# LittleWat/multichannel-semseg-with-uda

Hardware: AMD Instinct MI355X
Metric: RGB-D img/s (6x480x640) MCD train step, drn_d_38 (higher is better)
Workload: dtype f32 (operands split 2-way into scaled fp16, 3 cross terms on the fp16 MFMA pipe, fp32 accumulate)

## Files before the change

include/mcdseg.h:

```cpp
#ifndef MCDSEG_H
#define MCDSEG_H

#include <stddef.h>
#include <stdint.h>

#ifdef __cplusplus
extern "C" {
#endif
#pragma GCC visibility push(default)

#define MCDSEG_VERSION 101

int mcdseg_version(void);
const char* mcdseg_last_error(void);

#define MCDSEG_COMM_ID_BYTES 128
int mcdseg_comm_unique_id(void* id128);
int mcdseg_comm_init(void** comm, int32_t nranks, const void* id128, int32_t rank);
int mcdseg_comm_destroy(void* comm);
int mcdseg_allreduce(float* buf, int64_t count, void* comm, void* stream);

int32_t mcdseg_option_count(void);
const char* mcdseg_option_name(int32_t index);
int mcdseg_set_option(const char* name, int64_t value);
// ... 18 lines not shown
int mcdseg_conv_dgrad(const mcdseg_conv_desc* d, const float* dy, const float* wp_dgrad, float* dx, void* stream);
#define MCDSEG_MATH_F16X3 3
#define MCDSEG_MATH_BF16X6 6
#define MCDSEG_MATH_F16X1 1
int mcdseg_conv_split_packed_bytes(const mcdseg_conv_desc* d, int32_t math, int64_t* fprop_bytes, int64_t* dgrad_bytes);
int32_t mcdseg_conv_split_direct_ok(const mcdseg_conv_desc* d);
int64_t mcdseg_conv_split_stat_rows(const mcdseg_conv_desc* d);
int64_t mcdseg_conv_split_stat_rows_for(const mcdseg_conv_desc* d, int32_t math, int32_t presplit);
int32_t mcdseg_conv_split_window_ok(const mcdseg_conv_desc* d, int32_t math, int32_t presplit, int32_t dgrad);
int32_t mcdseg_conv_split_tile_config(int32_t M, int64_t P, int32_t presplit);
int mcdseg_absmax(const float* x, int64_t n, float* bound, void* stream);
int mcdseg_conv_split_pack_weights(const mcdseg_conv_desc* d, int32_t math, const float* w, void* wp_fprop, void* wp_dgrad,
                                   float* w_bound, void* stream);
int mcdseg_conv_split_pack_weights_multi(const int64_t* ptrs, const int32_t* dims, int32_t n, int32_t math, float* bounds,
                                         void* stream);
int mcdseg_conv_split_fprop(const mcdseg_conv_desc* d, int32_t math, const float* x, const void* x_cb, const float* x_bound,
                            const void* wp_fprop, const float* w_bound, const float* bias, float* y, float* stat_partials,
                            void* stream);
int mcdseg_conv_split_fprop_affine(const mcdseg_conv_desc* d, int32_t math, const float* x, const void* x_cb, const float* x_bound,
                                   const void* wp_fprop, const float* w_bound, const float* scale, const float* shift,
                                   const float* residual, int32_t relu, float* y, void* stream);
int mcdseg_conv_split_dgrad(const mcdseg_conv_desc* d, int32_t math, const float* dy, const void* dy_cb, const float* dy_bound,
                            const void* wp_dgrad, const float* w_bound, float* dx, void* stream);
int mcdseg_conv_split_dgrad_add(const mcdseg_conv_desc* d, int32_t math, const float* dy, const void* dy_cb, const float* dy_bound,
                                const void* wp_dgrad, const float* w_bound, const float* addend, float* dx, int32_t part, void* stream);
int64_t mcdseg_conv_split_parts(const mcdseg_conv_desc* d, int32_t math, int32_t presplit, int32_t dgrad);
int32_t mcdseg_conv_split_rest_pingpong(const mcdseg_conv_desc* d, int32_t math, int32_t presplit, int32_t dgrad);
int32_t mcdseg_conv_split_wide_pingpong(const mcdseg_conv_desc* d, int32_t math, int32_t presplit, int32_t dgrad);
int mcdseg_conv_split_fprop_part(const mcdseg_conv_desc* d, int32_t math, const float* x, const void* x_cb, const float* x_bound,
                                 const void* wp_fprop, const float* w_bound, const float* bias, float* y, float* stat_partials,
// ... 141 lines not shown
                         int32_t relu, void* stream);
size_t mcdseg_bn_bwd_half_workspace_bytes(int32_t N, int32_t C, int32_t HW);
int mcdseg_bn_bwd_reduce_half(const void* dy16, const void* y_cb, const void* z16, const float* z_bound, const float* mean,
                              const float* rstd, const float* gamma, const float* beta, float* dgamma, float* dbeta, float* dz_bound,
                              int32_t mask_kind, int32_t train, int32_t N, int32_t C, int32_t HW, void* workspace, size_t workspace_bytes,
                              void* stream);
int mcdseg_bn_bwd_apply_half(const void* dy16, const void* y_cb, const void* z16, const float* z_bound, const float* mean,
                             const float* rstd, const float* gamma, const float* beta, const float* dgamma, const float* dbeta, void* dz_cb,
                             const float* dz_bound, void* dres16, int32_t mask_kind, int32_t train, int32_t N, int32_t C, int32_t HW,
                             void* stream);
int mcdseg_pack_bf16_units(const float* x, void* out16, int32_t N, int32_t C, int32_t HW, void* stream);
int mcdseg_unpack_bf16_units(const void* in16, float* x, int32_t N, int32_t C, int32_t HW, void* stream);

int mcdseg_sgd_momentum_flat(float* p, const float* g, float* v, int64_t n, float lr, float momentum,
                             float weight_decay, float grad_scale, void* stream);

int mcdseg_adam_flat(float* p, const float* g, float* m, float* v, int64_t n, float lr_over_bc1, float beta1, float beta2,
                     float inv_sqrt_bc2, float eps, float weight_decay, float grad_scale, void* stream);

#pragma GCC visibility pop
#ifdef __cplusplus
}
#endif
#endif
```

multichannel-semseg-with-uda_amd/csrc/conv_gemm_split.hip:

```cpp
#include <cstdlib>
#include <type_traits>

#include "conv_split_params.h"
#include "options.h"

namespace {


template <class P, int WM, int WN, int WAVES_M, int WAVES_N, bool DGRAD, bool PRESPLIT>
__global__ __launch_bounds__(256, 2) void conv_gemm_split_kernel(ConvSplitParams p) {
  constexpr int BM = 32 * WM * WAVES_M;
  constexpr int BN = 32 * WN * WAVES_N;
  constexpr int NT = 256;
  static_assert(WAVES_M * WAVES_N == 4, "4 waves per workgroup");
  constexpr int B_ITEMS = BN * 2 / NT;
  constexpr int NP = P::NP;
  constexpr int NQ = 2 * NP;
  typedef typename P::frag frag;
  constexpr int A_CHUNKS = NQ * BM;
  constexpr int A_ITERS = (A_CHUNKS + NT - 1) / NT;
  constexpr bool A_EXACT = (A_CHUNKS % NT) == 0;
  constexpr bool A_DMA = A_EXACT;
  constexpr int A_ITERS_DMA = ((2 * P::NPU * BM) % NT == 0) ? (2 * P::NPU * BM) / NT : A_ITERS;
  constexpr int A_BYTES = NQ * BM * 16, B_BYTES = NQ * BN * 16;
// ... 679 lines not shown
      m = t > m ? t : m;
    }
    i += n4 << 2;
  }
  for (; i < n; i += step) {
    const unsigned b = __float_as_uint(x[i]) & 0x7FFFFFFFu;
    m = b > m ? b : m;
  }
  for (int o = 1; o < 64; o <<= 1) {
    const unsigned t = __shfl_xor(m, o);
    m = t > m ? t : m;
  }
  if ((threadIdx.x & 63) == 0 && m != 0u) atomicMax(out, m);
}

__global__ __launch_bounds__(256) void absmax_multi_kernel(const int64_t* __restrict__ ptrs, const int32_t* __restrict__ dims) {
  const int e = blockIdx.y;
  const float* __restrict__ x = reinterpret_cast<const float*>(ptrs[4 * e + 0]);
  unsigned* __restrict__ out = reinterpret_cast<unsigned*>(ptrs[4 * e + 3]);
  const int64_t n = (int64_t)dims[4 * e + 0] * dims[4 * e + 1] * dims[4 * e + 2];
  const int64_t step = (int64_t)gridDim.x * blockDim.x;
  unsigned m = 0u;
  int64_t i = blockIdx.x * (int64_t)blockDim.x + threadIdx.x;
  for (; i + 3 * step < n; i += 4 * step) {
    const unsigned b0 = __float_as_uint(x[i]) & 0x7FFFFFFFu, b1 = __float_as_uint(x[i + step]) & 0x7FFFFFFFu;
    const unsigned b2 = __float_as_uint(x[i + 2 * step]) & 0x7FFFFFFFu, b3 = __float_as_uint(x[i + 3 * step]) & 0x7FFFFFFFu;
    const unsigned c0 = b0 > b1 ? b0 : b1, c1 = b2 > b3 ? b2 : b3;
    const unsigned c = c0 > c1 ? c0 : c1;
    m = c > m ? c : m;
  }
  for (; i < n; i += step) {
    const unsigned b = __float_as_uint(x[i]) & 0x7FFFFFFFu;
    m = b > m ? b : m;
  }
  for (int o = 1; o < 64; o <<= 1) {
    const unsigned t = __shfl_xor(m, o);
    m = t > m ? t : m;
  }
  if ((threadIdx.x & 63) == 0 && m != 0u) atomicMax(out, m);
}

template <class P>
__global__ __launch_bounds__(256) void pack_weights_multi_kernel(const int64_t* __restrict__ ptrs, const int32_t* __restrict__ dims) {
  constexpr int NP = P::NP;
  __shared__ float tile[32 * 16 * 9 + 32];
  const int e = blockIdx.y >> 1, mode = blockIdx.y & 1;
  const float* __restrict__ w = reinterpret_cast<const float*>(ptrs[4 * e + 0]);
  typename P::elem* __restrict__ out = reinterpret_cast<typename P::elem*>(ptrs[4 * e + 1 + mode]);
  if (out == nullptr) return;
  const float inv_scale = 1.f / operand_scale<P>(reinterpret_cast<const float*>(ptrs[4 * e + 3]));
  const int Cout = dims[4 * e + 0], Cin = dims[4 * e + 1], T = dims[4 * e + 2];
  const int M = mode == 0 ? Cout : Cin;
  const int K = mode == 0 ? Cin : Cout;
  const int Mp = M <= 32 ? 32 : (M <= 64 ? 64 : ((M + 127) / 128) * 128);
  const int Kp = ((K + 15) / 16) * 16;
  const int MT = T <= 9 ? 32 : (T <= 18 ? 16 : (T <= 36 ? 8 : 4));
  const int row_len = 16 * T + 1;
  const int m_tiles = Mp / MT, chunks = Kp / 16;
  const int t = threadIdx.x;
  for (int tl = blockIdx.x; tl < m_tiles * chunks; tl += gridDim.x) {
    const int chunk = tl / m_tiles, m0 = (tl - chunk * m_tiles) * MT, k0 = chunk * 16;
    __syncthreads();
    if (mode == 0) {
      for (int idx = t; idx < MT * 16 * T; idx += 256) {
        const int mm = idx / (16 * T), col = idx - mm * (16 * T);
// ... 240 lines not shown
                       (__bf16*)wp_dgrad, (const float*)nullptr, d->Cout, d->Cin, T);
  MCD_LAUNCH_CHECK("conv_split_pack_weights");
  return 0;
}

extern "C" int mcdseg_conv_split_pack_weights_multi(const int64_t* ptrs, const int32_t* dims, int32_t n, int32_t math, float* bounds,
                                                    void* stream) {
  math = mcd_storage_math(math);
  MCD_REQUIRE(ptrs && dims && n > 0 && n <= 32767, "conv_split_pack_weights_multi: bad table");
  MCD_REQUIRE(math == MCDSEG_MATH_BF16X6 || math == MCDSEG_MATH_F16X3, "conv_split_pack_weights_multi: unknown math %d", math);
  MCD_REQUIRE(math != MCDSEG_MATH_F16X3 || bounds != nullptr, "conv_split_pack_weights_multi: f16x3 needs the bounds array");
  hipStream_t st = (hipStream_t)stream;
  const unsigned pack_blocks = (unsigned)(mcd_opt(MCD_OPT_PACK_BLOCKS) > 0 ? mcd_opt(MCD_OPT_PACK_BLOCKS) : 192);
  if (math == MCDSEG_MATH_F16X3) {
    (void)hipMemsetAsync(bounds, 0, sizeof(float) * (size_t)n, st);
    hipLaunchKernelGGL(absmax_multi_kernel, dim3(48, (unsigned)n), dim3(256), 0, st, ptrs, dims);
    MCD_LAUNCH_CHECK("absmax_multi");
    hipLaunchKernelGGL(pack_weights_multi_kernel<SplitF16x3>, dim3(pack_blocks, 2u * (unsigned)n), dim3(256), 0, st, ptrs, dims);
  } else {
    hipLaunchKernelGGL(pack_weights_multi_kernel<SplitBf16x6>, dim3(pack_blocks, 2u * (unsigned)n), dim3(256), 0, st, ptrs, dims);
  }
  MCD_LAUNCH_CHECK("conv_split_pack_weights_multi");
  return 0;
}

static int split_cb_bytes(const mcdseg_conv_desc* d, int math, int C, int HW, const void* cb, int* piece_bytes, long long* piece_stride) {
  *piece_bytes = 0;
  *piece_stride = 0;
  if (cb == nullptr) return 0;
  MCD_REQUIRE((C % 8) == 0, "conv_split: a pre-split operand needs a channel count divisible by 8 (got %d)", C);
  MCD_REQUIRE(d->Ncb == 0 || d->Ncb >= d->N, "conv_split: Ncb (%d) must be 0 or at least N (%d)", d->Ncb, d->N);
  const int64_t b = (int64_t)d->N * C * HW * 2;
  MCD_REQUIRE(b < (1ll << 31), "conv_split: one piece of the pre-split operand exceeds 2 GiB; split the batch");
  *piece_bytes = (int)b;
  *piece_stride = math == MCDSEG_MATH_F16X1 ? 0 : (long long)(d->Ncb ? d->Ncb : d->N) * C * HW * 2;
  return 0;
}

// ... 217 lines not shown
```

multichannel-semseg-with-uda_amd/csrc/sgd.hip:

```cpp
#include "common.h"

namespace {

__global__ __launch_bounds__(256) void sgd_momentum_kernel(float* __restrict__ p, const float* __restrict__ g, float* __restrict__ v,
                                                           int64_t n4, int64_t n, float lr, float mu, float wd, float gs) {
  float4* p4 = reinterpret_cast<float4*>(p);
  const float4* g4 = reinterpret_cast<const float4*>(g);
  float4* v4 = reinterpret_cast<float4*>(v);
  for (int64_t i = blockIdx.x * (int64_t)blockDim.x + threadIdx.x; i < n4; i += (int64_t)gridDim.x * blockDim.x) {
    float4 pp = p4[i];
    const float4 gg = g4[i];
    float4 vv = v4[i];
    vv.x = fmaf(mu, vv.x, fmaf(wd, pp.x, gg.x * gs));
    vv.y = fmaf(mu, vv.y, fmaf(wd, pp.y, gg.y * gs));
    vv.z = fmaf(mu, vv.z, fmaf(wd, pp.z, gg.z * gs));
    vv.w = fmaf(mu, vv.w, fmaf(wd, pp.w, gg.w * gs));
    pp.x = fmaf(-lr, vv.x, pp.x);
    pp.y = fmaf(-lr, vv.y, pp.y);
    pp.z = fmaf(-lr, vv.z, pp.z);
    pp.w = fmaf(-lr, vv.w, pp.w);
    v4[i] = vv;
    p4[i] = pp;
  }
  for (int64_t i = n4 * 4 + blockIdx.x * (int64_t)blockDim.x + threadIdx.x; i < n; i += (int64_t)gridDim.x * blockDim.x) {
// ... 6 lines not shown
}

extern "C" int mcdseg_sgd_momentum_flat(float* p, const float* g, float* v, int64_t n, float lr, float momentum, float weight_decay,
                                        float grad_scale, void* stream) {
  MCD_REQUIRE(p && g && v && n >= 0, "sgd_momentum_flat: bad arguments");
  if (n == 0) return 0;
  const bool al = ((reinterpret_cast<uintptr_t>(p) | reinterpret_cast<uintptr_t>(g) | reinterpret_cast<uintptr_t>(v)) & 15) == 0;
  const int64_t n4 = al ? n / 4 : 0;
  int64_t blocks = ceil_div64(n4 > 0 ? n4 : n, 256);
  if (blocks > 2048) blocks = 2048;
  hipLaunchKernelGGL(sgd_momentum_kernel, dim3((unsigned)blocks), dim3(256), 0, (hipStream_t)stream, p, g, v, n4, n, lr, momentum,
                     weight_decay, grad_scale);
  MCD_LAUNCH_CHECK("sgd_momentum_flat");
  return 0;
}
```

multichannel-semseg-with-uda_amd/mcdseg/_lib.py:

```python
import ctypes
import glob
import os
import subprocess
import threading

HERE = os.path.dirname(os.path.abspath(__file__))
PKG = os.path.dirname(HERE)
REPO = os.path.dirname(PKG)
CSRC = os.path.join(PKG, "csrc")
INCLUDE = os.path.join(REPO, "include")
LIB_PATH = os.environ.get("MCDSEG_LIB") or os.path.join(HERE, "libmcdseg.so")

c_void_p, c_int, c_i32, c_i64, c_float, c_size_t = (ctypes.c_void_p, ctypes.c_int, ctypes.c_int32, ctypes.c_int64,
                                                    ctypes.c_float, ctypes.c_size_t)


class ConvDesc(ctypes.Structure):
    _fields_ = [(n, c_i32) for n in ("N", "Cin", "H", "W", "Cout", "KH", "KW", "stride", "pad", "dil", "Ho", "Wo", "Ncb")]


_P = ctypes.POINTER
_SIGNATURES = {
    "mcdseg_version": (c_int, []),
    "mcdseg_last_error": (ctypes.c_char_p, []),
# ... 13 lines not shown
    "mcdseg_conv_split_window_ok": (c_i32, [_P(ConvDesc), c_i32, c_i32, c_i32]),
    "mcdseg_conv_split_direct_ok": (c_i32, [_P(ConvDesc)]),
    "mcdseg_conv_split_tile_config": (c_i32, [c_i32, c_i64, c_i32]),
    "mcdseg_conv_fprop": (c_int, [_P(ConvDesc), c_void_p, c_void_p, c_void_p, c_void_p, c_void_p, c_void_p]),
    "mcdseg_conv_fprop_affine": (c_int, [_P(ConvDesc), c_void_p, c_void_p, c_void_p, c_void_p, c_void_p, c_i32, c_void_p, c_void_p]),
    "mcdseg_bn_eval_affine": (c_int, [c_void_p] * 5 + [c_i32, c_float, c_void_p, c_void_p, c_void_p]),
    "mcdseg_predict_workspace_bytes": (c_size_t, [c_i32, c_i32]),
    "mcdseg_predict_labels": (c_int, [c_void_p] * 4 + [c_i32] * 4 + [c_void_p, c_size_t, c_void_p]),
    "mcdseg_predict_up8_workspace_bytes": (c_size_t, [c_i32, c_i32]),
    "mcdseg_predict_labels_up8": (c_int, [c_void_p] * 4 + [c_i32] * 5 + [c_void_p, c_size_t, c_void_p]),
    "mcdseg_depth_image_u8": (c_int, [c_void_p, c_void_p] + [c_i32] * 4 + [c_void_p]),
    "mcdseg_absmax": (c_int, [c_void_p, c_i64, c_void_p, c_void_p]),
    "mcdseg_conv_split_packed_bytes": (c_int, [_P(ConvDesc), c_i32, _P(c_i64), _P(c_i64)]),
    "mcdseg_conv_split_pack_weights": (c_int, [_P(ConvDesc), c_i32] + [c_void_p] * 5),
    "mcdseg_conv_split_pack_weights_multi": (c_int, [c_void_p, c_void_p, c_i32, c_i32, c_void_p, c_void_p]),
    "mcdseg_conv_split_fprop": (c_int, [_P(ConvDesc), c_i32] + [c_void_p] * 9),
    "mcdseg_conv_split_fprop_affine": (c_int, [_P(ConvDesc), c_i32] + [c_void_p] * 8 + [c_i32, c_void_p, c_void_p]),
    "mcdseg_conv_split_dgrad": (c_int, [_P(ConvDesc), c_i32] + [c_void_p] * 7),
    "mcdseg_conv_split_parts": (c_i64, [_P(ConvDesc), c_i32, c_i32, c_i32]),
    "mcdseg_conv_split_rest_pingpong": (c_i32, [_P(ConvDesc), c_i32, c_i32, c_i32]),
    "mcdseg_conv_split_wide_pingpong": (c_i32, [_P(ConvDesc), c_i32, c_i32, c_i32]),
    "mcdseg_conv_split_fprop_part": (c_int, [_P(ConvDesc), c_i32] + [c_void_p] * 8 + [c_i32, c_void_p]),
    "mcdseg_conv_split_dgrad_part": (c_int, [_P(ConvDesc), c_i32] + [c_void_p] * 6 + [c_i32, c_void_p]),
    "mcdseg_conv_split_dgrad_add": (c_int, [_P(ConvDesc), c_i32] + [c_void_p] * 7 + [c_i32, c_void_p]),
    "mcdseg_split_cb": (c_int, [c_void_p, c_void_p, c_void_p, c_i32, c_i32, c_i32, c_i32, c_void_p]),
    "mcdseg_split_cb_padded": (c_int, [c_void_p, c_void_p, c_void_p, c_i32, c_i32, c_i32, c_i32, c_void_p]),
    "mcdseg_unsplit_cb": (c_int, [c_void_p, c_void_p, c_i32, c_i32, c_i32, c_i32, c_void_p, c_void_p]),
    "mcdseg_bn_apply_cb": (c_int, [c_void_p] * 11 + [c_i32] * 5 + [c_void_p]),
    "mcdseg_bn_bwd_apply_cb": (c_int, [c_void_p] * 13 + [c_i32] * 6 + [c_void_p]),
    "mcdseg_bn_bwd_reduce_zmask": (c_int, [c_void_p] * 9 + [c_i32] * 4 + [c_void_p, c_size_t, c_void_p]),
# ... 41 lines not shown
    "mcdseg_gate_mix_fwd": (c_int, [c_void_p] * 4 + [c_i64, c_void_p]),
    "mcdseg_gate_mix_bwd": (c_int, [c_void_p] * 7 + [c_i64, c_void_p]),
    "mcdseg_softmax_ch_fwd": (c_int, [c_void_p, c_void_p, c_i32, c_i32, c_i32, c_void_p]),
    "mcdseg_softmax_ch_bwd": (c_int, [c_void_p, c_void_p, c_void_p, c_i32, c_i32, c_i32, c_void_p]),
    "mcdseg_prob_nll_workspace_bytes": (c_size_t, [c_i32, c_i32]),
    "mcdseg_prob_nll": (c_int, [c_void_p, c_void_p, c_void_p, c_i64, c_i32, c_void_p, c_void_p, c_i32, c_i32, c_i32, c_void_p,
                                c_size_t, c_void_p]),
    "mcdseg_normalize_u8": (c_int, [c_void_p] * 4 + [c_i32] * 6 + [c_void_p]),
    "mcdseg_resize_workspace_bytes": (c_size_t, [c_i32] * 6),
    "mcdseg_resize_bilinear_u8": (c_int, [c_void_p, c_void_p] + [c_i32] * 6 + [c_void_p, c_size_t, c_void_p]),
    "mcdseg_resize_nearest_u8": (c_int, [c_void_p, c_void_p] + [c_i32] * 5 + [c_void_p, c_size_t, c_void_p]),
    "mcdseg_relabel_u8": (c_int, [c_void_p, c_void_p, c_i64, c_i32, c_i32, c_void_p]),
    "mcdseg_confusion_hist": (c_int, [c_void_p, c_void_p, c_i64, c_i32, c_void_p, c_void_p]),
    "mcdseg_scale_by_device_scalar": (c_int, [c_void_p, c_void_p, c_i64, c_void_p]),
    "mcdseg_sgd_momentum_flat": (c_int, [c_void_p, c_void_p, c_void_p, c_i64, c_float, c_float, c_float, c_float, c_void_p]),
    "mcdseg_adam_flat": (c_int, [c_void_p] * 4 + [c_i64] + [c_float] * 7 + [c_void_p]),
    "mcdseg_conv_split_half_ok": (c_i32, [_P(ConvDesc), c_i32, c_i32]),
    "mcdseg_conv_split_pp_deep": (c_i32, [_P(ConvDesc), c_i32, c_i32]),
    "mcdseg_up8_loss_variant": (c_i32, [c_i32] * 5),
    "mcdseg_conv_wgrad_thin_tr_config": (c_i32, [_P(ConvDesc)]),
    "mcdseg_conv_split_fprop_half": (c_int, [_P(ConvDesc), c_i32] + [c_void_p] * 7 + [c_i32, c_void_p]),
    "mcdseg_conv_split_dgrad_half": (c_int, [_P(ConvDesc), c_i32] + [c_void_p] * 6 + [c_i32, c_void_p]),
    "mcdseg_bn_apply_half": (c_int, [c_void_p] * 10 + [c_i32] * 4 + [c_void_p]),
    "mcdseg_bn_bwd_half_workspace_bytes": (c_size_t, [c_i32] * 3),
    "mcdseg_bn_bwd_reduce_half": (c_int, [c_void_p] * 11 + [c_i32] * 5 + [c_void_p, c_size_t, c_void_p]),
    "mcdseg_bn_bwd_apply_half": (c_int, [c_void_p] * 13 + [c_i32] * 5 + [c_void_p]),
    "mcdseg_pack_bf16_units": (c_int, [c_void_p, c_void_p, c_i32, c_i32, c_i32, c_void_p]),
    "mcdseg_unpack_bf16_units": (c_int, [c_void_p, c_void_p, c_i32, c_i32, c_i32, c_void_p]),
}
EXPORTS = tuple(_SIGNATURES)
# ... 302 lines not shown
```

multichannel-semseg-with-uda_amd/mcdseg/ops.py:

```python
import collections
import contextlib
import ctypes
import os
import threading
import types
import weakref

import torch

from . import _lib
from ._lib import ConvDesc, check, get_option, lib

WEIGHT_EPOCH = 0


def bump_weight_epoch(params=None):
    global WEIGHT_EPOCH
    if params is None:
        WEIGHT_EPOCH += 1
        return
    for p in params:
        p._mcd_epoch = getattr(p, "_mcd_epoch", 0) + 1


# ... 234 lines not shown
        return bound
    rec = getattr(x, "_mcd_bound", None)
    if rec is not None and rec[1] == x._version and rec[2] == x.data_ptr():
        return rec[0]
    b = absmax(x)
    try:
        x._mcd_bound = (b, x._version, x.data_ptr())
    except AttributeError:
        pass
    return b


_PACK_REGISTRY = weakref.WeakSet()
_PACK_TABLES = {}
GROUP_PACK = os.environ.get("MCDSEG_GROUP_PACK", "1") != "0"
FUSED_UP_LOSS = os.environ.get("MCDSEG_FUSED_UP_LOSS", "1") != "0"
BN_ZMASK = os.environ.get("MCDSEG_BN_ZMASK", "1") != "0"
RELU_MASK = os.environ.get("MCDSEG_RELU_MASK", "1") != "0"
FUSE_RES_ADD = os.environ.get("MCDSEG_FUSE_RES_ADD", "1") != "0"


class GradBox:
    __slots__ = ("n", "seen", "g", "task")

    def __init__(self):
        self.n, self.seen, self.g, self.task = 0, 0, None, None

    def attach(self):
        self.n += 1
        return self
# ... 90 lines not shown

def _pack_group(device):
    L = lib()
    members = []
    for pw in list(_PACK_REGISTRY):
        w = pw._weight() if pw._weight is not None else None
        if (w is None or pw._dims is None or pw._dims[4] != CONV_MATH or w.device != device or pw.wd is None or pw.wf is None
                or pw._dims[2] > 72):
            continue
        members.append((pw, w))
    if len(members) < 2:
        return
    members.sort(key=lambda m: m[1].data_ptr())
    sig = tuple((w.data_ptr(), pw.wf.data_ptr(), pw.wd.data_ptr()) + pw._dims for pw, w in members)
    tab = _PACK_TABLES.get((device, CONV_MATH))
    if tab is None or tab["sig"] != sig:
        n = len(members)
        bounds = torch.zeros(n, dtype=torch.float32, device=device)
        ptrs, dims = [], []
        for i, (pw, w) in enumerate(members):
            ptrs += [w.data_ptr(), pw.wf.data_ptr(), pw.wd.data_ptr(), bounds.data_ptr() + 4 * i]
            dims += [pw._dims[0], pw._dims[1], pw._dims[2], 0]
        tab = dict(sig=sig, bounds=bounds, ptrs=torch.tensor(ptrs, dtype=torch.int64).to(device),
                   dims=torch.tensor(dims, dtype=torch.int32).to(device))
        _PACK_TABLES[(device, CONV_MATH)] = tab
    if _scaled():
        for i, (pw, _) in enumerate(members):
            pw.w_bound = tab["bounds"][i:i + 1]
    n = len(members)
    nbytes = sum(4 * w.numel() + 2 * pw.wf.numel() + 2 * pw.wd.numel() for pw, w in members)
    with _timed("pack_weights_multi_kernel", (0, nbytes)):
        check(L.mcdseg_conv_split_pack_weights_multi(_p(tab["ptrs"]), _p(tab["dims"]), n, MATH_ID[CONV_MATH],
                                                     _p(tab["bounds"]) if _scaled() else None, _stream()), "conv_split_pack_weights_multi")
    for pw, w in members:
        if pw._dims[3]:
            d = ConvDesc(1, pw._dims[1], 8, 8, pw._dims[0], 7, 7, 1, 3, 1, 8, 8)
            check(L.mcdseg_conv_split_pack_weights(ctypes.byref(d), MATH_ID[CONV_MATH], _p(w.detach()), _p(pw.wf), None,
                                                   _p(pw.w_bound) if _scaled() else None, _stream()), "conv_split_pack_weights")
        pw.key = PackedWeights._key_of(w)


def _is_split(w_image):
    return w_image.dtype == torch.int16


MAX_CONV_BYTES = int(os.environ.get("MCDSEG_MAX_CONV_BYTES", str((1 << 31) - (1 << 26))))


def _sub_desc(desc, n, ncb=0):
    return ConvDesc(n, desc.Cin, desc.H, desc.W, desc.Cout, desc.KH, desc.KW, desc.stride, desc.pad, desc.dil, desc.Ho, desc.Wo, ncb)


def _cb_slice(cb, a, channels, hw):
    return None if cb is None else ctypes.c_void_p(cb.data_ptr() + a * (channels // 8) * hw * 16)
# ... 1412 lines not shown
    if kind == 0:
        return _Diff2d.apply(z1, z2)
    return _ProbDistance.apply(z1, z2, kind)


def sgd_momentum_flat_(p, g, v, lr, momentum, weight_decay, grad_scale=1.0, params=None):
    for t, name in ((p, "params"), (g, "grads"), (v, "momentum")):
        if not (t.is_cuda and t.dtype == torch.float32 and t.is_contiguous()):
            raise RuntimeError("mcdseg: flat SGD needs contiguous fp32 GPU buffers (%s)" % name)
    with _timed("sgd_momentum_kernel", (0, 20 * p.numel())):
        check(lib().mcdseg_sgd_momentum_flat(_p(p), _p(g), _p(v), p.numel(), float(lr), float(momentum), float(weight_decay),
                                             float(grad_scale), _stream()), "sgd_momentum_flat")
    bump_weight_epoch(params)


def adam_flat_(p, g, m, v, lr, betas, eps, weight_decay, step, grad_scale=1.0, params=None):
    for t, name in ((p, "params"), (g, "grads"), (m, "exp_avg"), (v, "exp_avg_sq")):
        if not (t.is_cuda and t.dtype == torch.float32 and t.is_contiguous()):
            raise RuntimeError("mcdseg: flat Adam needs contiguous fp32 GPU buffers (%s)" % name)
    b1, b2 = float(betas[0]), float(betas[1])
    step = int(step)
    if step < 1:
        raise ValueError("mcdseg: flat Adam's step count starts at 1, got %r" % (step,))
    bc1, bc2 = 1.0 - b1 ** step, 1.0 - b2 ** step
    with _timed("adam_kernel", (0, 28 * p.numel())):
        check(lib().mcdseg_adam_flat(_p(p), _p(g), _p(m), _p(v), p.numel(), float(lr) / bc1, b1, b2, bc2 ** -0.5, float(eps),
                                     float(weight_decay), float(grad_scale), _stream()), "adam_flat")
    bump_weight_epoch(params)
```

multichannel-semseg-with-uda_amd/mcdseg/optim.py:

```python
import os

import torch

from . import dist as mdist
from . import ops

_ALIGN = 64
DP_OVERLAP = os.environ.get("MCDSEG_DP_OVERLAP", "0") == "1"
DP_BUCKET_MB = float(os.environ.get("MCDSEG_DP_BUCKET_MB", "25"))


class _FlatOptimizer(torch.optim.Optimizer):
    _require_gpu = True
    _STATE = ()

    def __init__(self, params, defaults):
        super().__init__(params, defaults)
        self._flat = None

    @property
    def _name(self):
        return type(self).__name__

    def _all_params(self):
# ... 208 lines not shown
                cur = None
                continue
            key = self._run_key(g, p)
            if cur is None or cur["key"] != key:
                cur = dict(key=key, params=[])
                runs.append(cur)
            cur["params"].append(p)
        world = mdist.world_size()
        for run in runs:
            ps = run["params"]
            o0 = fl["views"][id(ps[0])][0]
            o1, n1 = fl["views"][id(ps[-1])][0], fl["views"][id(ps[-1])][1]
            lo, hi = o0, o1 + n1
            gflat = fl["g"][lo:hi]
            reduced = bool(fl.get("buckets")) and self._finish_overlap(ps)
            if not reduced:
                gviews = [fl["views"][id(p)][3] for p in ps]
                grads = [p.grad if p.grad.dtype == torch.float32 else p.grad.float() for p in ps]
                torch._foreach_copy_(gviews, grads)
                if mdist.is_distributed():
                    mdist.all_reduce_sum_(gflat)
            self._update(fl, lo, hi, gflat, run["key"], ps, 1.0 / world)
        self._reset_overlap()
        return loss

    def zero_grad(self, set_to_none=True):
        super().zero_grad(set_to_none=set_to_none)
        if self._flat is not None:
            self._reset_overlap()

    def state_dict(self):
        sd = super().state_dict()
        sd["state"] = {k: {name: (t.clone() if torch.is_tensor(t) else t) for name, t in st.items()} for k, st in sd["state"].items()}
        return sd

    def load_state_dict(self, state_dict):
        super().load_state_dict(state_dict)
        names = {name for _, name in self._STATE}
        for st in self.state.values():
            st.update((name, t.clone()) for name, t in list(st.items()) if torch.is_tensor(t) and (name not in names or self._flat is None))
        if self._flat is not None:
            self._adopt_state()

    def flat_buffers(self):
        self._ensure_flat()
        return (self._flat["p"], self._flat["g"]) + tuple(self._flat[key] for key, _ in self._STATE)

    def _run_key(self, group, p):
        raise NotImplementedError

    def _update(self, fl, lo, hi, gflat, key, ps, grad_scale):
        raise NotImplementedError


class FlatSGD(_FlatOptimizer):
    _STATE = (("v", "momentum_buffer"),)

    def __init__(self, params, lr=1e-3, momentum=0.0, weight_decay=0.0):
        if lr < 0 or momentum < 0 or weight_decay < 0:
            raise ValueError("FlatSGD: negative hyper-parameter")
        super().__init__(params, dict(lr=lr, momentum=momentum, weight_decay=weight_decay, dampening=0, nesterov=False))

    def _run_key(self, group, p):
        return (group["lr"], group["momentum"], group["weight_decay"])

    def _update(self, fl, lo, hi, gflat, key, ps, grad_scale):
        lr, mu, wd = key
        ops.sgd_momentum_flat_(fl["p"][lo:hi], gflat, fl["v"][lo:hi], lr, mu, wd, grad_scale, params=ps)
        if mu != 0:
            for p in ps:
                self.state[p]["momentum_buffer"] = fl["views"][id(p)][2]

    def flat_buffers(self):
        return super().flat_buffers()


class FlatAdam(_FlatOptimizer):
    _STATE = (("m", "exp_avg"), ("v", "exp_avg_sq"))

    def __init__(self, params, lr=1e-3, betas=(0.9, 0.999), eps=1e-8, weight_decay=0.0, amsgrad=False, maximize=False):
        if amsgrad or maximize:
            raise NotImplementedError("FlatAdam: amsgrad and maximize are not implemented")
        if lr < 0 or eps < 0 or weight_decay < 0 or not (0 <= betas[0] < 1 and 0 <= betas[1] < 1):
            raise ValueError("FlatAdam: negative hyper-parameter, or a beta outside [0, 1)")
        super().__init__(params, dict(lr=lr, betas=tuple(betas), eps=eps, weight_decay=weight_decay, amsgrad=False, maximize=False,
                                      foreach=None, capturable=False, differentiable=False, fused=None, decoupled_weight_decay=False))

    def _run_key(self, group, p):
        if group.get("amsgrad") or group.get("maximize") or group.get("decoupled_weight_decay"):
            raise NotImplementedError("FlatAdam: amsgrad, maximize and decoupled weight decay are not implemented")
        st = self.state[p]
        if "step" not in st:
            m, v = self._state_views(p)
            st.update(step=torch.tensor(0.0, dtype=torch.float32), exp_avg=m, exp_avg_sq=v)
        elif not torch.is_tensor(st["step"]):
            st["step"] = torch.tensor(float(st["step"]), dtype=torch.float32)
        return (float(group["lr"]), tuple(group["betas"]), group["eps"], group["weight_decay"], int(st["step"]) + 1)

    def _update(self, fl, lo, hi, gflat, key, ps, grad_scale):
        lr, betas, eps, wd, t = key
        ops.adam_flat_(fl["p"][lo:hi], gflat, fl["m"][lo:hi], fl["v"][lo:hi], lr, betas, eps, wd, t, grad_scale, params=ps)
        torch._foreach_add_([self.state[p]["step"] for p in ps], 1)
```

Before: 82.82.

## Fuse weight abs-max bound into SGD update and read gradients in place

Adds a segmented SGD momentum kernel that reads each parameter's gradient directly, with no copy into the flat buffer, and atomically records the abs-max of the updated weights into double-buffered bound slots. The weight packer can then reuse these measured bounds and skip its separate abs-max pass for weights the optimizer just updated. It also repacks only the weights that changed. This removes a foreach gradient copy and a full reread of the weights for the bound, at the cost of extra host-side bookkeeping (dirty sets, selection tables, pinned table uploads) and a more complex, fragile caching protocol.

```diff
diff --git a/include/mcdseg.h b/include/mcdseg.h
--- a/include/mcdseg.h
+++ b/include/mcdseg.h
@@ -56,6 +56,9 @@
                                    float* w_bound, void* stream);
 int mcdseg_conv_split_pack_weights_multi(const int64_t* ptrs, const int32_t* dims, int32_t n, int32_t math, float* bounds,
                                          void* stream);
+int mcdseg_conv_split_pack_weights_bounded(const int64_t* ptrs, const int32_t* dims, int32_t n, int32_t math, const int32_t* sel,
+                                           int32_t n_sel, int32_t n_measure, const float* measured, float* clear, void* stream);
+int mcdseg_conv_split_pack_stem_image(const mcdseg_conv_desc* d, int32_t math, const float* w, void* wp_fprop, void* stream);
 int mcdseg_conv_split_fprop(const mcdseg_conv_desc* d, int32_t math, const float* x, const void* x_cb, const float* x_bound,
                             const void* wp_fprop, const float* w_bound, const float* bias, float* y, float* stat_partials,
                             void* stream);
@@ -227,6 +230,9 @@
 
 int mcdseg_sgd_momentum_flat(float* p, const float* g, float* v, int64_t n, float lr, float momentum,
                              float weight_decay, float grad_scale, void* stream);
+int32_t mcdseg_sgd_segment_chunk(void);
+int mcdseg_sgd_momentum_segments(float* p, float* v, const int64_t* segments, int32_t n_segments, const int32_t* blocks, int64_t n_blocks,
+                                 float lr, float momentum, float weight_decay, float grad_scale, void* stream);
 
 int mcdseg_adam_flat(float* p, const float* g, float* m, float* v, int64_t n, float lr_over_bc1, float beta1, float beta2,
                      float inv_sqrt_bc2, float eps, float weight_decay, float grad_scale, void* stream);
diff --git a/multichannel-semseg-with-uda_amd/csrc/conv_gemm_split.hip b/multichannel-semseg-with-uda_amd/csrc/conv_gemm_split.hip
--- a/multichannel-semseg-with-uda_amd/csrc/conv_gemm_split.hip
+++ b/multichannel-semseg-with-uda_amd/csrc/conv_gemm_split.hip
@@ -717,8 +717,9 @@
   if ((threadIdx.x & 63) == 0 && m != 0u) atomicMax(out, m);
 }
 
-__global__ __launch_bounds__(256) void absmax_multi_kernel(const int64_t* __restrict__ ptrs, const int32_t* __restrict__ dims) {
-  const int e = blockIdx.y;
+__global__ __launch_bounds__(256) void absmax_multi_kernel(const int64_t* __restrict__ ptrs, const int32_t* __restrict__ dims,
+                                                           const int32_t* __restrict__ idx) {
+  const int e = idx != nullptr ? idx[blockIdx.y] : (int)blockIdx.y;
   const float* __restrict__ x = reinterpret_cast<const float*>(ptrs[4 * e + 0]);
   unsigned* __restrict__ out = reinterpret_cast<unsigned*>(ptrs[4 * e + 3]);
   const int64_t n = (int64_t)dims[4 * e + 0] * dims[4 * e + 1] * dims[4 * e + 2];
@@ -744,14 +745,24 @@
 }
 
 template <class P>
-__global__ __launch_bounds__(256) void pack_weights_multi_kernel(const int64_t* __restrict__ ptrs, const int32_t* __restrict__ dims) {
+__global__ __launch_bounds__(256) void pack_weights_multi_kernel(const int64_t* __restrict__ ptrs, const int32_t* __restrict__ dims,
+                                                                 const int32_t* __restrict__ idx, int n_measure,
+                                                                 const float* __restrict__ measured, float* __restrict__ clear, int n_clear) {
   constexpr int NP = P::NP;
   __shared__ float tile[32 * 16 * 9 + 32];
-  const int e = blockIdx.y >> 1, mode = blockIdx.y & 1;
+  const int j = blockIdx.y >> 1, mode = blockIdx.y & 1;
+  const int e = idx != nullptr ? idx[j] : j;
+  if (clear != nullptr && blockIdx.x == 0 && blockIdx.y == 0)
+    for (int i = threadIdx.x; i < n_clear; i += 256) clear[i] = 0.f;
   const float* __restrict__ w = reinterpret_cast<const float*>(ptrs[4 * e + 0]);
   typename P::elem* __restrict__ out = reinterpret_cast<typename P::elem*>(ptrs[4 * e + 1 + mode]);
+  const float* __restrict__ bound = reinterpret_cast<const float*>(ptrs[4 * e + 3]);
+  if (idx != nullptr && j >= n_measure && measured != nullptr) {
+    bound = measured + e;
+    if (blockIdx.x == 0 && mode == 0 && threadIdx.x == 0) *reinterpret_cast<float*>(ptrs[4 * e + 3]) = *bound;
+  }
   if (out == nullptr) return;
-  const float inv_scale = 1.f / operand_scale<P>(reinterpret_cast<const float*>(ptrs[4 * e + 3]));
+  const float inv_scale = 1.f / operand_scale<P>(bound);
   const int Cout = dims[4 * e + 0], Cin = dims[4 * e + 1], T = dims[4 * e + 2];
   const int M = mode == 0 ? Cout : Cin;
   const int K = mode == 0 ? Cin : Cout;
@@ -1022,14 +1033,63 @@
   const unsigned pack_blocks = (unsigned)(mcd_opt(MCD_OPT_PACK_BLOCKS) > 0 ? mcd_opt(MCD_OPT_PACK_BLOCKS) : 192);
   if (math == MCDSEG_MATH_F16X3) {
     (void)hipMemsetAsync(bounds, 0, sizeof(float) * (size_t)n, st);
-    hipLaunchKernelGGL(absmax_multi_kernel, dim3(48, (unsigned)n), dim3(256), 0, st, ptrs, dims);
+    hipLaunchKernelGGL(absmax_multi_kernel, dim3(48, (unsigned)n), dim3(256), 0, st, ptrs, dims, (const int32_t*)nullptr);
     MCD_LAUNCH_CHECK("absmax_multi");
-    hipLaunchKernelGGL(pack_weights_multi_kernel<SplitF16x3>, dim3(pack_blocks, 2u * (unsigned)n), dim3(256), 0, st, ptrs, dims);
+    hipLaunchKernelGGL(pack_weights_multi_kernel<SplitF16x3>, dim3(pack_blocks, 2u * (unsigned)n), dim3(256), 0, st, ptrs, dims,
+                       (const int32_t*)nullptr, 0, (const float*)nullptr, (float*)nullptr, 0);
   } else {
-    hipLaunchKernelGGL(pack_weights_multi_kernel<SplitBf16x6>, dim3(pack_blocks, 2u * (unsigned)n), dim3(256), 0, st, ptrs, dims);
+    hipLaunchKernelGGL(pack_weights_multi_kernel<SplitBf16x6>, dim3(pack_blocks, 2u * (unsigned)n), dim3(256), 0, st, ptrs, dims,
+                       (const int32_t*)nullptr, 0, (const float*)nullptr, (float*)nullptr, 0);
   }
   MCD_LAUNCH_CHECK("conv_split_pack_weights_multi");
   return 0;
+}
+
+__global__ void zero_bounds_kernel(const int64_t* __restrict__ ptrs, const int32_t* __restrict__ idx, int n) {
+  const int j = blockIdx.x * blockDim.x + threadIdx.x;
+  if (j < n) *reinterpret_cast<float*>(ptrs[4 * idx[j] + 3]) = 0.f;
+}
+
+extern "C" int mcdseg_conv_split_pack_weights_bounded(const int64_t* ptrs, const int32_t* dims, int32_t n, int32_t math, const int32_t* sel,
+                                                      int32_t n_sel, int32_t n_measure, const float* measured, float* clear,
+                                                      void* stream) {
+  math = mcd_storage_math(math);
+  MCD_REQUIRE(ptrs && dims && n > 0 && n <= 32767, "conv_split_pack_weights_bounded: bad table");
+  MCD_REQUIRE(math == MCDSEG_MATH_BF16X6 || math == MCDSEG_MATH_F16X3, "conv_split_pack_weights_bounded: unknown math %d", math);
+  MCD_REQUIRE(n_sel >= 0 && n_sel <= n && n_measure >= 0 && n_measure <= n_sel && (n_sel == 0 || sel != nullptr),
+              "conv_split_pack_weights_bounded: bad selection (%d of %d entries, %d to measure)", (int)n_sel, (int)n, (int)n_measure);
+  MCD_REQUIRE(math != MCDSEG_MATH_F16X3 || n_measure == n_sel || measured != nullptr,
+              "conv_split_pack_weights_bounded: entries with a measured bound need the array that holds it");
+  MCD_REQUIRE(clear == nullptr || clear != measured, "conv_split_pack_weights_bounded: the array to clear is the one being read");
+  hipStream_t st = (hipStream_t)stream;
+  if (n_sel == 0) {
+    if (clear != nullptr) (void)hipMemsetAsync(clear, 0, sizeof(float) * (size_t)n, st);
+    MCD_LAUNCH_CHECK("conv_split_pack_weights_bounded");
+    return 0;
+  }
+  const unsigned pack_blocks = (unsigned)(mcd_opt(MCD_OPT_PACK_BLOCKS) > 0 ? mcd_opt(MCD_OPT_PACK_BLOCKS) : 192);
+  if (math == MCDSEG_MATH_F16X3) {
+    if (n_measure > 0) {
+      hipLaunchKernelGGL(zero_bounds_kernel, dim3((unsigned)ceil_div64(n_measure, 256)), dim3(256), 0, st, ptrs, sel, (int)n_measure);
+      hipLaunchKernelGGL(absmax_multi_kernel, dim3(48, (unsigned)n_measure), dim3(256), 0, st, ptrs, dims, sel);
+      MCD_LAUNCH_CHECK("absmax_multi");
+    }
+    hipLaunchKernelGGL(pack_weights_multi_kernel<SplitF16x3>, dim3(pack_blocks, 2u * (unsigned)n_sel), dim3(256), 0, st, ptrs, dims, sel,
+                       (int)n_measure, measured, clear, (int)n);
+  } else {
+    hipLaunchKernelGGL(pack_weights_multi_kernel<SplitBf16x6>, dim3(pack_blocks, 2u * (unsigned)n_sel), dim3(256), 0, st, ptrs, dims, sel,
+                       (int)n_sel, (const float*)nullptr, clear, (int)n);
+  }
+  MCD_LAUNCH_CHECK("conv_split_pack_weights_bounded");
+  return 0;
+}
+
+extern "C" int mcdseg_conv_split_pack_stem_image(const mcdseg_conv_desc* d, int32_t math, const float* w, void* wp_fprop, void* stream) {
+  math = mcd_storage_math(math);
+  if (int rc = split_check(d, math, "conv_split_pack_stem_image", false)) return rc;
+  MCD_REQUIRE(w != nullptr && wp_fprop != nullptr, "conv_split_pack_stem_image: null pointer");
+  MCD_REQUIRE(mcdseg_internal_stem_ok(d), "conv_split_pack_stem_image: not a geometry of the direct stem kernel");
+  return mcdseg_internal_stem_pack(d, w, (char*)wp_fprop + stem_image_offset(d, math), (hipStream_t)stream);
 }
 
 static int split_cb_bytes(const mcdseg_conv_desc* d, int math, int C, int HW, const void* cb, int* piece_bytes, long long* piece_stride) {
diff --git a/multichannel-semseg-with-uda_amd/csrc/sgd.hip b/multichannel-semseg-with-uda_amd/csrc/sgd.hip
--- a/multichannel-semseg-with-uda_amd/csrc/sgd.hip
+++ b/multichannel-semseg-with-uda_amd/csrc/sgd.hip
@@ -44,3 +44,106 @@
   MCD_LAUNCH_CHECK("sgd_momentum_flat");
   return 0;
 }
+
+#define MCD_SGD_CHUNK 4096
+
+namespace {
+
+__device__ __forceinline__ unsigned sgd_update4(float4& pp, const float4 gg, float4& vv, float lr, float mu, float wd, float gs) {
+  vv.x = fmaf(mu, vv.x, fmaf(wd, pp.x, gg.x * gs));
+  vv.y = fmaf(mu, vv.y, fmaf(wd, pp.y, gg.y * gs));
+  vv.z = fmaf(mu, vv.z, fmaf(wd, pp.z, gg.z * gs));
+  vv.w = fmaf(mu, vv.w, fmaf(wd, pp.w, gg.w * gs));
+  pp.x = fmaf(-lr, vv.x, pp.x);
+  pp.y = fmaf(-lr, vv.y, pp.y);
+  pp.z = fmaf(-lr, vv.z, pp.z);
+  pp.w = fmaf(-lr, vv.w, pp.w);
+  const unsigned a = __float_as_uint(pp.x) & 0x7FFFFFFFu, b = __float_as_uint(pp.y) & 0x7FFFFFFFu;
+  const unsigned c = __float_as_uint(pp.z) & 0x7FFFFFFFu, d = __float_as_uint(pp.w) & 0x7FFFFFFFu;
+  const unsigned ab = a > b ? a : b, cd = c > d ? c : d;
+  return ab > cd ? ab : cd;
+}
+
+__global__ __launch_bounds__(256) void sgd_momentum_seg_kernel(float* __restrict__ p, float* __restrict__ v, const int64_t* __restrict__ seg,
+                                                               int nseg, const int32_t* __restrict__ blocks, float lr, float mu, float wd,
+                                                               float gs) {
+  __shared__ unsigned wave_max[4];
+  const int s = blocks[2 * blockIdx.x], chunk = blocks[2 * blockIdx.x + 1];
+  if (s < 0 || s >= nseg || chunk < 0) return;
+  const int64_t n = seg[4 * s + 1], lo = (int64_t)chunk * MCD_SGD_CHUNK;
+  if (lo >= n) return;
+  const int cnt = (int)(n - lo < MCD_SGD_CHUNK ? n - lo : MCD_SGD_CHUNK);
+  float* __restrict__ pc = p + seg[4 * s + 0] + lo;
+  float* __restrict__ vc = v + seg[4 * s + 0] + lo;
+  const float* __restrict__ gc = reinterpret_cast<const float*>(seg[4 * s + 2]) + lo;
+  unsigned* __restrict__ slot = reinterpret_cast<unsigned*>(seg[4 * s + 3]);
+  const int t = threadIdx.x;
+  unsigned m = 0u;
+  int done = 0;
+  if (((reinterpret_cast<uintptr_t>(pc) | reinterpret_cast<uintptr_t>(vc) | reinterpret_cast<uintptr_t>(gc)) & 15) == 0) {
+    float4* __restrict__ p4 = reinterpret_cast<float4*>(pc);
+    float4* __restrict__ v4 = reinterpret_cast<float4*>(vc);
+    const float4* __restrict__ g4 = reinterpret_cast<const float4*>(gc);
+    const int n4 = cnt >> 2;
+    if (n4 == MCD_SGD_CHUNK / 4) {
+      float4 pp[4], gg[4], vv[4];
+#pragma unroll
+      for (int j = 0; j < 4; ++j) {
+        pp[j] = p4[t + 256 * j];
+        gg[j] = g4[t + 256 * j];
+        vv[j] = v4[t + 256 * j];
+      }
+#pragma unroll
+      for (int j = 0; j < 4; ++j) {
+        const unsigned a = sgd_update4(pp[j], gg[j], vv[j], lr, mu, wd, gs);
+        m = a > m ? a : m;
+        v4[t + 256 * j] = vv[j];
+        p4[t + 256 * j] = pp[j];
+      }
+    } else {
+      for (int i = t; i < n4; i += 256) {
+        float4 pp = p4[i], vv = v4[i];
+        const unsigned a = sgd_update4(pp, g4[i], vv, lr, mu, wd, gs);
+        m = a > m ? a : m;
+        v4[i] = vv;
+        p4[i] = pp;
+      }
+    }
+    done = n4 << 2;
+  }
+  for (int i = done + t; i < cnt; i += 256) {
+    const float vv = fmaf(mu, vc[i], fmaf(wd, pc[i], gc[i] * gs));
+    const float pn = fmaf(-lr, vv, pc[i]);
+    vc[i] = vv;
+    pc[i] = pn;
+    const unsigned a = __float_as_uint(pn) & 0x7FFFFFFFu;
+    m = a > m ? a : m;
+  }
+  if (slot == nullptr) return;
+  for (int o = 1; o < 64; o <<= 1) {
+    const unsigned x = __shfl_xor(m, o);
+    m = x > m ? x : m;
+  }
+  if ((t & 63) == 0) wave_max[t >> 6] = m;
+  __syncthreads();
+  if (t == 0) {
+    const unsigned a = wave_max[0] > wave_max[1] ? wave_max[0] : wave_max[1], b = wave_max[2] > wave_max[3] ? wave_max[2] : wave_max[3];
+    const unsigned r = a > b ? a : b;
+    if (r != 0u) atomicMax(slot, r);
+  }
+}
+
+}
+
+extern "C" int32_t mcdseg_sgd_segment_chunk(void) { return MCD_SGD_CHUNK; }
+
+extern "C" int mcdseg_sgd_momentum_segments(float* p, float* v, const int64_t* segments, int32_t n_segments, const int32_t* blocks,
+                                            int64_t n_blocks, float lr, float momentum, float weight_decay, float grad_scale, void* stream) {
+  MCD_REQUIRE(p && v && segments && blocks, "sgd_momentum_segments: null pointer");
+  MCD_REQUIRE(n_segments > 0 && n_blocks > 0 && n_blocks <= 0x7FFFFFFFll, "sgd_momentum_segments: bad table sizes (%d segments, %lld blocks)",
+              (int)n_segments, (long long)n_blocks);
+  hipLaunchKernelGGL(sgd_momentum_seg_kernel, dim3((unsigned)n_blocks), dim3(256), 0, (hipStream_t)stream, p, v, segments, (int)n_segments,
+                     blocks, lr, momentum, weight_decay, grad_scale);
+  MCD_LAUNCH_CHECK("sgd_momentum_segments");
+  return 0;
+}
diff --git a/multichannel-semseg-with-uda_amd/mcdseg/_lib.py b/multichannel-semseg-with-uda_amd/mcdseg/_lib.py
--- a/multichannel-semseg-with-uda_amd/mcdseg/_lib.py
+++ b/multichannel-semseg-with-uda_amd/mcdseg/_lib.py
@@ -51,6 +51,8 @@
     "mcdseg_conv_split_packed_bytes": (c_int, [_P(ConvDesc), c_i32, _P(c_i64), _P(c_i64)]),
     "mcdseg_conv_split_pack_weights": (c_int, [_P(ConvDesc), c_i32] + [c_void_p] * 5),
     "mcdseg_conv_split_pack_weights_multi": (c_int, [c_void_p, c_void_p, c_i32, c_i32, c_void_p, c_void_p]),
+    "mcdseg_conv_split_pack_weights_bounded": (c_int, [c_void_p, c_void_p, c_i32, c_i32, c_void_p, c_i32, c_i32, c_void_p, c_void_p, c_void_p]),
+    "mcdseg_conv_split_pack_stem_image": (c_int, [_P(ConvDesc), c_i32, c_void_p, c_void_p, c_void_p]),
     "mcdseg_conv_split_fprop": (c_int, [_P(ConvDesc), c_i32] + [c_void_p] * 9),
     "mcdseg_conv_split_fprop_affine": (c_int, [_P(ConvDesc), c_i32] + [c_void_p] * 8 + [c_i32, c_void_p, c_void_p]),
     "mcdseg_conv_split_dgrad": (c_int, [_P(ConvDesc), c_i32] + [c_void_p] * 7),
@@ -122,6 +124,8 @@
     "mcdseg_confusion_hist": (c_int, [c_void_p, c_void_p, c_i64, c_i32, c_void_p, c_void_p]),
     "mcdseg_scale_by_device_scalar": (c_int, [c_void_p, c_void_p, c_i64, c_void_p]),
     "mcdseg_sgd_momentum_flat": (c_int, [c_void_p, c_void_p, c_void_p, c_i64, c_float, c_float, c_float, c_float, c_void_p]),
+    "mcdseg_sgd_segment_chunk": (c_i32, []),
+    "mcdseg_sgd_momentum_segments": (c_int, [c_void_p] * 3 + [c_i32, c_void_p, c_i64] + [c_float] * 4 + [c_void_p]),
     "mcdseg_adam_flat": (c_int, [c_void_p] * 4 + [c_i64] + [c_float] * 7 + [c_void_p]),
     "mcdseg_conv_split_half_ok": (c_i32, [_P(ConvDesc), c_i32, c_i32]),
     "mcdseg_conv_split_pp_deep": (c_i32, [_P(ConvDesc), c_i32, c_i32]),
diff --git a/multichannel-semseg-with-uda_amd/mcdseg/ops.py b/multichannel-semseg-with-uda_amd/mcdseg/ops.py
--- a/multichannel-semseg-with-uda_amd/mcdseg/ops.py
+++ b/multichannel-semseg-with-uda_amd/mcdseg/ops.py
@@ -272,6 +272,8 @@
 _PACK_REGISTRY = weakref.WeakSet()
 _PACK_TABLES = {}
 GROUP_PACK = os.environ.get("MCDSEG_GROUP_PACK", "1") != "0"
+SGD_BOUNDS = os.environ.get("MCDSEG_SGD_BOUNDS", "1") != "0"
+_TABLE_SERIAL = [0]
 FUSED_UP_LOSS = os.environ.get("MCDSEG_FUSED_UP_LOSS", "1") != "0"
 BN_ZMASK = os.environ.get("MCDSEG_BN_ZMASK", "1") != "0"
 RELU_MASK = os.environ.get("MCDSEG_RELU_MASK", "1") != "0"
@@ -392,30 +394,63 @@
     members.sort(key=lambda m: m[1].data_ptr())
     sig = tuple((w.data_ptr(), pw.wf.data_ptr(), pw.wd.data_ptr()) + pw._dims for pw, w in members)
     tab = _PACK_TABLES.get((device, CONV_MATH))
-    if tab is None or tab["sig"] != sig:
-        n = len(members)
+    fresh = tab is None or tab["sig"] != sig
+    n = len(members)
+    if fresh:
         bounds = torch.zeros(n, dtype=torch.float32, device=device)
         ptrs, dims = [], []
         for i, (pw, w) in enumerate(members):
             ptrs += [w.data_ptr(), pw.wf.data_ptr(), pw.wd.data_ptr(), bounds.data_ptr() + 4 * i]
             dims += [pw._dims[0], pw._dims[1], pw._dims[2], 0]
+        _TABLE_SERIAL[0] += 1
         tab = dict(sig=sig, bounds=bounds, ptrs=torch.tensor(ptrs, dtype=torch.int64).to(device),
-                   dims=torch.tensor(dims, dtype=torch.int32).to(device))
+                   dims=torch.tensor(dims, dtype=torch.int32).to(device), serial=_TABLE_SERIAL[0],
+                   acc=torch.zeros(2, n, dtype=torch.float32, device=device), cur=0, dirty=[set(), set()], rec={},
+                   index={id(w): i for i, (_, w) in enumerate(members)}, sel={})
         _PACK_TABLES[(device, CONV_MATH)] = tab
     if _scaled():
         for i, (pw, _) in enumerate(members):
             pw.w_bound = tab["bounds"][i:i + 1]
-    n = len(members)
-    nbytes = sum(4 * w.numel() + 2 * pw.wf.numel() + 2 * pw.wd.numel() for pw, w in members)
+    if not SGD_BOUNDS:
+        nbytes = sum(4 * w.numel() + 2 * pw.wf.numel() + 2 * pw.wd.numel() for pw, w in members)
+        with _timed("pack_weights_multi_kernel", (0, nbytes)):
+            check(L.mcdseg_conv_split_pack_weights_multi(_p(tab["ptrs"]), _p(tab["dims"]), n, MATH_ID[CONV_MATH],
+                                                         _p(tab["bounds"]) if _scaled() else None, _stream()), "conv_split_pack_weights_multi")
+        for pw, w in members:
+            if pw._dims[3]:
+                d = ConvDesc(1, pw._dims[1], 8, 8, pw._dims[0], 7, 7, 1, 3, 1, 8, 8)
+                check(L.mcdseg_conv_split_pack_weights(ctypes.byref(d), MATH_ID[CONV_MATH], _p(w.detach()), _p(pw.wf), None,
+                                                       _p(pw.w_bound) if _scaled() else None, _stream()), "conv_split_pack_weights")
+            pw.key = PackedWeights._key_of(w)
+        return
+    keys = [PackedWeights._key_of(w) for _, w in members]
+    rec, cur = tab["rec"], tab["cur"]
+    measure, known = [], []
+    for i, ((pw, _), key) in enumerate(zip(members, keys)):
+        if not fresh and pw.key == key:
+            continue
+        (known if (_scaled() and rec.get(i) == key) else measure).append(i)
+    pattern = (tuple(measure), tuple(known))
+    sel = tab["sel"].get(pattern)
+    if sel is None:
+        if len(tab["sel"]) >= 16:
+            tab["sel"].clear()
+        sel = tab["sel"][pattern] = torch.tensor(measure + known + [0], dtype=torch.int32).to(device)
+    nbytes = sum(4 * members[i][1].numel() + 2 * members[i][0].wf.numel() + 2 * members[i][0].wd.numel() for i in measure + known)
     with _timed("pack_weights_multi_kernel", (0, nbytes)):
-        check(L.mcdseg_conv_split_pack_weights_multi(_p(tab["ptrs"]), _p(tab["dims"]), n, MATH_ID[CONV_MATH],
-                                                     _p(tab["bounds"]) if _scaled() else None, _stream()), "conv_split_pack_weights_multi")
-    for pw, w in members:
+        check(L.mcdseg_conv_split_pack_weights_bounded(_p(tab["ptrs"]), _p(tab["dims"]), n, MATH_ID[CONV_MATH], _p(sel),
+                                                       len(measure) + len(known), len(measure), _p(tab["acc"][cur]),
+                                                       _p(tab["acc"][1 - cur]), _stream()), "conv_split_pack_weights_bounded")
+    tab["dirty"][1 - cur].clear()
+    tab["cur"] = 1 - cur
+    rec.clear()
+    for i in measure + known:
+        pw, w = members[i]
         if pw._dims[3]:
             d = ConvDesc(1, pw._dims[1], 8, 8, pw._dims[0], 7, 7, 1, 3, 1, 8, 8)
-            check(L.mcdseg_conv_split_pack_weights(ctypes.byref(d), MATH_ID[CONV_MATH], _p(w.detach()), _p(pw.wf), None,
-                                                   _p(pw.w_bound) if _scaled() else None, _stream()), "conv_split_pack_weights")
-        pw.key = PackedWeights._key_of(w)
+            check(L.mcdseg_conv_split_pack_stem_image(ctypes.byref(d), MATH_ID[CONV_MATH], _p(w.detach()), _p(pw.wf), _stream()),
+                  "conv_split_pack_stem_image")
+        pw.key = keys[i]
 
 
 def _is_split(w_image):
@@ -1858,6 +1893,55 @@
     bump_weight_epoch(params)
 
 
+def sgd_momentum_segments_(p, v, segments, grads, params, lr, momentum, weight_decay, grad_scale, cache):
+    for t, name in ((p, "params"), (v, "momentum")) + tuple((g, "a gradient") for g in grads):
+        if not (t.is_cuda and t.dtype == torch.float32 and t.is_contiguous()):
+            raise RuntimeError("mcdseg: flat SGD needs contiguous fp32 GPU buffers (%s)" % name)
+    if not (len(segments) == len(grads) == len(params)) or any(g.numel() != n for g, (_, n) in zip(grads, segments)):
+        raise ValueError("mcdseg: flat SGD: segments, gradients and parameters do not match")
+    L, dev = lib(), p.device
+    tab = _PACK_TABLES.get((dev, CONV_MATH)) if (_scaled() and GROUP_PACK) else None
+    slots, cur, acc_ptr = None, 0, 0
+    if tab is not None:
+        slots = [tab["index"].get(id(q), -1) for q in params]
+        cur = tab["cur"]
+        dirty = tab["dirty"][cur]
+        if any(i in dirty for i in slots):
+            tab["acc"][cur].zero_()
+            dirty.clear()
+            tab["rec"].clear()
+        acc_ptr = tab["acc"][cur].data_ptr()
+    if "blocks" not in cache:
+        chunk = L.mcdseg_sgd_segment_chunk()
+        rows = [torch.stack((torch.full((c,), i, dtype=torch.int32), torch.arange(c, dtype=torch.int32)), 1)
+                for i, c in enumerate((n + chunk - 1) // chunk for _, n in segments)]
+        cache["blocks"] = torch.cat(rows).contiguous().to(dev)
+        cache["tables"] = collections.OrderedDict()
+    gptrs = tuple(g.data_ptr() for g in grads)
+    key = (gptrs, tab["serial"] if tab is not None else 0, cur)
+    table = cache["tables"].get(key)
+    if table is None:
+        if len(cache["tables"]) >= 16:
+            cache["tables"].popitem(last=False)
+        rows = [[o, n, g, (acc_ptr + 4 * slots[i]) if (slots is not None and slots[i] >= 0) else 0]
+                for i, ((o, n), g) in enumerate(zip(segments, gptrs))]
+        table = cache["tables"][key] = torch.tensor(rows, dtype=torch.int64).pin_memory().to(dev, non_blocking=True)
+        SGD_TABLE_UPLOADS[0] += 1
+    blocks = cache["blocks"]
+    with _timed("sgd_momentum_seg_kernel", (0, 20 * sum(n for _, n in segments))):
+        check(L.mcdseg_sgd_momentum_segments(_p(p), _p(v), _p(table), len(segments), _p(blocks), blocks.shape[0], float(lr), float(momentum),
+                                             float(weight_decay), float(grad_scale), _stream()), "sgd_momentum_segments")
+    bump_weight_epoch(params)
+    if tab is not None:
+        for q, i in zip(params, slots):
+            if i >= 0:
+                dirty.add(i)
+                tab["rec"][i] = PackedWeights._key_of(q)
+
+
+SGD_TABLE_UPLOADS = [0]
+
+
 def adam_flat_(p, g, m, v, lr, betas, eps, weight_decay, step, grad_scale=1.0, params=None):
     for t, name in ((p, "params"), (g, "grads"), (m, "exp_avg"), (v, "exp_avg_sq")):
         if not (t.is_cuda and t.dtype == torch.float32 and t.is_contiguous()):
diff --git a/multichannel-semseg-with-uda_amd/mcdseg/optim.py b/multichannel-semseg-with-uda_amd/mcdseg/optim.py
--- a/multichannel-semseg-with-uda_amd/mcdseg/optim.py
+++ b/multichannel-semseg-with-uda_amd/mcdseg/optim.py
@@ -246,13 +246,15 @@
             lo, hi = o0, o1 + n1
             gflat = fl["g"][lo:hi]
             reduced = bool(fl.get("buckets")) and self._finish_overlap(ps)
-            if not reduced:
+            direct = (not reduced and self._reads_grads_in_place(fl) and not mdist.is_distributed()
+                      and all(p.grad.dtype == torch.float32 and p.grad.is_contiguous() for p in ps))
+            if not reduced and not direct:
                 gviews = [fl["views"][id(p)][3] for p in ps]
                 grads = [p.grad if p.grad.dtype == torch.float32 else p.grad.float() for p in ps]
                 torch._foreach_copy_(gviews, grads)
                 if mdist.is_distributed():
                     mdist.all_reduce_sum_(gflat)
-            self._update(fl, lo, hi, gflat, run["key"], ps, 1.0 / world)
+            self._update(fl, lo, hi, gflat, run["key"], ps, 1.0 / world, in_place=direct)
         self._reset_overlap()
         return loss
 
@@ -281,8 +283,11 @@
     def _run_key(self, group, p):
         raise NotImplementedError
 
-    def _update(self, fl, lo, hi, gflat, key, ps, grad_scale):
+    def _update(self, fl, lo, hi, gflat, key, ps, grad_scale, in_place=False):
         raise NotImplementedError
+
+    def _reads_grads_in_place(self, fl):
+        return False
 
 
 class FlatSGD(_FlatOptimizer):
@@ -296,9 +301,21 @@
     def _run_key(self, group, p):
         return (group["lr"], group["momentum"], group["weight_decay"])
 
-    def _update(self, fl, lo, hi, gflat, key, ps, grad_scale):
+    def _reads_grads_in_place(self, fl):
+        return ops.SGD_BOUNDS and fl["p"].is_cuda
+
+    def _segments(self, ps):
+        views = self._flat["views"]
+        return [views[id(p)][:2] for p in ps]
+
+    def _update(self, fl, lo, hi, gflat, key, ps, grad_scale, in_place=False):
         lr, mu, wd = key
-        ops.sgd_momentum_flat_(fl["p"][lo:hi], gflat, fl["v"][lo:hi], lr, mu, wd, grad_scale, params=ps)
+        if self._reads_grads_in_place(fl):
+            cache = fl.setdefault("seg", {}).setdefault((id(ps[0]), id(ps[-1]), len(ps)), {})
+            grads = [p.grad for p in ps] if in_place else [fl["views"][id(p)][3] for p in ps]
+            ops.sgd_momentum_segments_(fl["p"], fl["v"], self._segments(ps), grads, ps, lr, mu, wd, grad_scale, cache)
+        else:
+            ops.sgd_momentum_flat_(fl["p"][lo:hi], gflat, fl["v"][lo:hi], lr, mu, wd, grad_scale, params=ps)
         if mu != 0:
             for p in ps:
                 self.state[p]["momentum_buffer"] = fl["views"][id(p)][2]
@@ -329,7 +346,7 @@
             st["step"] = torch.tensor(float(st["step"]), dtype=torch.float32)
         return (float(group["lr"]), tuple(group["betas"]), group["eps"], group["weight_decay"], int(st["step"]) + 1)
 
-    def _update(self, fl, lo, hi, gflat, key, ps, grad_scale):
+    def _update(self, fl, lo, hi, gflat, key, ps, grad_scale, in_place=False):
         lr, betas, eps, wd, t = key
         ops.adam_flat_(fl["p"][lo:hi], gflat, fl["m"][lo:hi], fl["v"][lo:hi], lr, betas, eps, wd, t, grad_scale, params=ps)
         torch._foreach_add_([self.state[p]["step"] for p in ps], 1)
```

After: 83.20, median of 6. No clear change (+0.5%).
